# facebookresearch/sylph-few-shot-detection

Hardware: AMD Instinct MI355X
Metric: query images/sec, R50-FPN 5-way 5-shot 800x1333 (whole job) (higher is better)
Workload: dtype bf16

## Files before the change

include/sylph_hip.h:

```cpp
#ifndef SYLPH_HIP_H
#define SYLPH_HIP_H

#include <stdint.h>

#ifdef __cplusplus
extern "C" {
#endif

typedef struct sylph_ctx sylph_ctx;

enum { SYLPH_F32 = 0, SYLPH_BF16 = 1, SYLPH_F32S = 2 };

typedef struct sylph_config {
  int resnet_depth;
  int stride_in_1x1;
  int num_cls_convs;
  int num_box_convs;
  int nlevels;
  int strides[8];
  float pixel_mean[3];
  float pixel_std[3];
  int size_divisibility;
  int use_scale;
  int cond_use_bias;
// ... 60 lines not shown
int sylph_export_head(sylph_ctx* ctx, int level, float* logits_nchw_dev, float* reg_nchw_dev, float* ctr_nchw_dev,
                      float* iou_nchw_dev);

int sylph_import_head(sylph_ctx* ctx, int N, int level, const float* logits_nchw_dev, const float* reg_nchw_dev,
                      const float* ctr_nchw_dev, const float* iou_nchw_dev);

int sylph_decode_nms(sylph_ctx* ctx, const int* out_heights, const int* out_widths, int max_out, float* boxes_dev,
                     float* scores_dev, int* classes_dev, int* levels_dev, float* locations_dev, int* cand_dev,
                     int* counts_dev, int* status_dev);

int sylph_codegen(sylph_ctx* ctx, const float* boxes_dev, float* code_out_dev);
int sylph_codegen_classes(sylph_ctx* ctx, const float* boxes_dev, int shots, float* codes_out_dev);
int sylph_codegen_rois(sylph_ctx* ctx, int R, const float* boxes_dev, const int* roi_image, int n_seg, const int* seg_len,
                       float* codes_out_dev);
int sylph_roi_table_uploads(sylph_ctx* ctx, int64_t* n_out);
int sylph_codegen_weight_norm(sylph_ctx* ctx, float* weight_norm_out_dev);

int sylph_roi_align(sylph_ctx* ctx, const float* boxes_dev, float* out_nchw_dev);
int sylph_roi_align_rois(sylph_ctx* ctx, int R, const float* boxes_dev, const int* roi_image, float* out_nchw_dev);

int sylph_normalize_codes(sylph_ctx* ctx, float* codes_dev, int n, const float* weight_norm_dev);

int sylph_reduce_codes(sylph_ctx* ctx, const float* rows_dev, int n, int row_ld, float* out_dev, int num_classes,
                       int divide_by_acc);

int sylph_allgather_codes(sylph_ctx* ctx, void* comm, const float* local_dev, int n_local, int capacity, float* out_dev);
int sylph_comm_unique_id(char* id_out_128);
int sylph_comm_init_rank(sylph_ctx* ctx, const char* id_128, int nranks, int rank, void** comm_out);
int sylph_comm_destroy(void* comm);

int sylph_conv2d(sylph_ctx* ctx, const float* x_nchw_dev, int B, int C, int H, int W, const float* w_host, int Cout,
                 int KH, int KW, int stride, int pad, const float* scale_host, const float* shift_host, int relu,
                 const float* residual_nchw_dev, float* y_nchw_dev);
int sylph_group_norm(sylph_ctx* ctx, const float* x_nchw_dev, int B, int H, int W, const float* gamma_host,
                     const float* beta_host, int relu, float* y_nchw_dev);

int sylph_stem_maxpool(sylph_ctx* ctx, const float* x_nchw_dev, int B, int H, int W, const float* w_host,
                       const float* scale_host, const float* shift_host, float* stem_out_nchw_dev, float* pool_out_nchw_dev);

int sylph_set_debug_taps(sylph_ctx* ctx, int on);
int sylph_export_stage(sylph_ctx* ctx, int stage, float* out_nchw_dev);
int sylph_export_tower(sylph_ctx* ctx, int tower, int layer, int level, float* y_nchw_dev, float* coef_dev);

#define SYLPH_SUP_ROI 0
#define SYLPH_SUP_GN_Y 1
#define SYLPH_SUP_GN_COEF 2
#define SYLPH_SUP_LAYER_OUT 3
#define SYLPH_SUP_CONV_OUT 4
#define SYLPH_SUP_CONTEXT 5
#define SYLPH_SUP_MSCAM 6
#define SYLPH_SUP_TOKENS 7
#define SYLPH_SUP_CLS_TOKENS 8
int sylph_support_tap_numel(sylph_ctx* ctx, int stage, int index, int64_t* numel);
int sylph_export_support(sylph_ctx* ctx, int stage, int index, float* out_dev);

int sylph_bottleneck(sylph_ctx* ctx, const float* x_nchw_dev, int B, int Cin, int H, int W, int stride, int mid, int cout,
                     const float* const* w_host, const float* const* scale_host, const float* const* shift_host,
                     float* y_nchw_dev);
int sylph_bottleneck_even(sylph_ctx* ctx, const float* x_nchw_dev, int B, int Cin, int H, int W, int mid, int cout,
                          const float* const* w_host, const float* const* scale_host, const float* const* shift_host,
                          float* y_nchw_dev);

int sylph_fpn_lateral(sylph_ctx* ctx, const float* x_nchw_dev, int B, int C, int H, int W, const float* w_host, const float* bias_host,
                      const float* top_nchw_dev, float* y_nchw_dev);

int sylph_group_conv(sylph_ctx* ctx, const float* x_nchw_dev, int B, int C, int H, int W, int groups, int stride, const float* w_host,
// ... 24 lines not shown
```

sylph-few-shot-detection_amd/csrc/api_conv.hip:

```cpp
#include "api_internal.h"

namespace sylph_host {

void level_dims(const sylph_config& cfg, int H, int W, int* hl, int* wl, int* off, int* Ltot) {
  int h = H / 8, w = W / 8;
  int o = 0;
  for (int l = 0; l < cfg.nlevels; ++l) {
    hl[l] = h; wl[l] = w; off[l] = o;
    o += h * w;
    if (l < 2) { h = (h - 1) / 2 + 1; w = (w - 1) / 2 + 1; }
    else { h = (h + 1) / 2; w = (w + 1) / 2; }
  }
  *Ltot = o;
}

int make_geom(sylph_ctx* c, const std::vector<SegDesc>& segs, int BM, Geom* g) {
  std::vector<int2> tiles;
  for (size_t s = 0; s < segs.size(); ++s) {
    const int rows = segs[s].out_H * segs[s].out_W;
    const int t0 = (int)tiles.size();
    for (int r = 0; r < rows; r += BM) tiles.push_back(make_int2((int)s, r));
    g->seg_tiles.push_back(make_int2(t0, (int)tiles.size() - t0));
  }
  void *ds = nullptr, *dtl = nullptr;
  RET(upload(c, &ds, segs.data(), segs.size() * sizeof(SegDesc)));
  RET(upload(c, &dtl, tiles.data(), tiles.size() * sizeof(int2)));
  g->segs = (const SegDesc*)ds;
  g->tiles = (const int2*)dtl;
  g->n_mtiles = (int)tiles.size();
  return 0;
}

void pick_patch(int H, int W, int max_pos, int halo_rows, int xpad, int* ph_out, int* pw_out) {
  long best_n = -1;
  int bh = 8, bw = 16, best_halo = 0;
  for (int w = 4; w <= 32; ++w) {
    for (int h = 1; h * w <= max_pos; ++h) {
      if ((h + 2) * (w + xpad) > halo_rows) continue;
      if (((max_pos - 1) / w + 2) * (w + xpad) + (max_pos - 1) % w + 2 >= halo_rows) continue;
      const long n = (long)((H + h - 1) / h) * ((W + w - 1) / w);
      const int halo = (h + 2) * (w + 2);
      const bool better = best_n < 0 || n < best_n || (n == best_n && (halo < best_halo || (halo == best_halo && w == 16)));
      if (better) { best_n = n; bh = h; bw = w; best_halo = halo; }
    }
  }
  *ph_out = bh; *pw_out = bw;
}

void set_patch(SegDesc* s, int ph, int pw, int xpad) {
  s->ph = ph; s->pw = pw; s->hpitch = pw + xpad;
  s->inv_pw = (65536u + pw - 1) / pw;
  s->inv_hw2 = (65536u + s->hpitch - 1) / s->hpitch;
}

int make_geom_patch(sylph_ctx* c, std::vector<SegDesc> segs, int max_pos, int halo_rows, int xpad, bool pair, Geom* g, int group) {
  std::vector<int2> tiles;
  if (group < 1 || segs.size() % (size_t)group != 0) group = 1;
  size_t g0 = 0;
  bool per_image = pair && segs.size() < (1u << 20);
  for (size_t s = 0; s < segs.size(); ++s) {
    int ph, pw;
    pick_patch(segs[s].out_H, segs[s].out_W, max_pos, halo_rows, xpad, &ph, &pw);
    set_patch(&segs[s], ph, pw, xpad);
    const int t0 = (int)tiles.size();
    for (int y = 0; y < segs[s].out_H; y += ph)
      for (int x = 0; x < segs[s].out_W; x += pw) tiles.push_back(make_int2((int)s, (y << 16) | x));
    g->seg_tiles.push_back(make_int2(t0, (int)tiles.size() - t0));
    if (per_image && (s + 1) % (size_t)group == 0) {
      const size_t n = tiles.size() - g0;
      if ((n & 1) && n < 8) per_image = false;
      if (per_image) {
        if (n & 1) tiles.push_back(make_int2(0, 0x7fff << 16));
        for (size_t t = g0; t < tiles.size(); t += 2) tiles[t].x |= (int)((((t - g0) >> 1) & 0x7ff) << 20);
      }
      g0 = tiles.size();
    }
  }
  if (pair && (tiles.size() & 1)) tiles.push_back(make_int2(0, 0x7fff << 16));
  if (pair && !per_image)
    for (size_t t = 0; t < tiles.size(); t += 2) tiles[t].x |= (int)(((t >> 1) & 0x7ff) << 20);
  g->n_mtiles = (int)tiles.size();
  void *ds = nullptr, *dtl = nullptr;
  RET(upload(c, &ds, segs.data(), segs.size() * sizeof(SegDesc)));
  RET(upload(c, &dtl, tiles.data(), tiles.size() * sizeof(int2)));
  g->segs = (const SegDesc*)ds;
  g->tiles = (const int2*)dtl;
  return 0;
}

long patch_count(const std::vector<SegDesc>& segs, int max_pos, int halo_rows, int xpad) {
  long n = 0;
  for (auto& sg : segs) {
    int ph, pw;
    pick_patch(sg.out_H, sg.out_W, max_pos, halo_rows, xpad, &ph, &pw);
    n += (long)((sg.out_H + ph - 1) / ph) * ((sg.out_W + pw - 1) / pw);
  }
  return n;
}

int timed_op(sylph_ctx* c, const char* kern, double flops, hipStream_t s, const std::function<int(hipStream_t)>& fn) {
  if (!c->prof) return fn(s);
  sylph_ctx::ProfRec r;
  if (!c->prof_free.empty()) {
    r.a = c->prof_free.back().first; r.b = c->prof_free.back().second;
    c->prof_free.pop_back();
  } else {
    if (hipEventCreate(&r.a) != hipSuccess || hipEventCreate(&r.b) != hipSuccess) return -100;
  }
  r.flops = flops;
  r.kern = kern;
  (void)hipEventRecord(r.a, s);
  const int rc = fn(s);
  (void)hipEventRecord(r.b, s);
  c->prof_recs.push_back(r);
  return rc;
}

static long total_rows(const std::vector<SegDesc>& segs) {
// ... 172 lines not shown
      gsegs[i].out_row0 = r0;
      r0 += n;
      max_rows = std::max(max_rows, n);
    }
  }
  Geom g;
  if (kind == ConvKind::hpipe) RET(make_geom_patch(c, segs, 128, 256, 4, true, &g, o.segs_per_image));
  else if (kind == ConvKind::igemm_halo) RET(make_geom_patch(c, segs, 128, 184, 2, false, &g));
  else RET(make_geom(c, gsegs, BM, &g));
  ConvArgs a;
  memset(&a, 0, sizeof(a));
  a.halo = kind == ConvKind::igemm_halo;
  a.nbuf2 = r.nbuf;
  a.in = in; a.wt = L.w; a.out = out; a.res = o.res;
  if (!igemm) RET(packed_weights(c, L, r, &a));
  if (pw) {
    std::vector<PwDesc> pd;
    for (const SegDesc& sg : segs) {
      const int nrows = sg.out_H * sg.out_W;
      for (int r0 = 0; r0 < nrows; r0 += BM) {
        PwDesc d;
        memset(&d, 0, sizeof(d));
        d.row0 = r0; d.seg_rows = nrows; d.out_W = sg.out_W; d.out_row0 = sg.out_row0; d.in_row0 = sg.in_row0; d.in_W = sg.in_W;
        d.in2_row0 = sg.in2_row0; d.in2_W = o.in2 ? sg.in2_W : sg.out_W; d.res_row0 = sg.res_row0; d.res_W = sg.res_W;
        pd.push_back(d);
      }
    }
    if ((int)pd.size() != g.n_mtiles) return fail("internal: conv_pw descriptor count");
    void* pdd = nullptr;
    RET(upload(c, &pdd, pd.data(), pd.size() * sizeof(PwDesc)));
    a.pw_desc = (const PwDesc*)pdd;
  }
  a.scale = L.scale; a.shift = L.shift; a.zeros = c->zeros;
  a.segs = g.segs; a.tiles = g.tiles; a.n_mtiles = kind == ConvKind::hpipe ? (g.n_mtiles + 1) / 2 : g.n_mtiles; a.n_ntiles = L.Cout_pad / BN;
  a.Cin = L.Cin; a.Cout = o.cout_override >= 0 ? o.cout_override : L.Cout;
  a.KH = L.KH; a.KW = L.KW; a.stride = o.stride; a.pad = o.pad;
  a.in_ld = in_ld; a.out_ld = out_ld; a.res_ld = o.res_ld;
  a.relu_nch = o.relu_nch; a.mul_nch = o.mul_nch; a.res_mode = o.res_mode;
  a.stem = o.stem; a.tap_dy = o.stem ? L.Cin / 32 : 1;
  a.gn_coef = o.gn_coef; a.gn_relu = o.gn_relu;
  a.ss_padded = 1;
  if (o.in2) {
    a.in2 = o.in2; a.in2_ld = o.in2_ld; a.Cin2 = o.Cin2; a.stride2 = o.stride2;
    a.Cin = L.Cin - o.Cin2;
  }
  if (o.want_gn) {
    if (L.Cout != 256 && L.Cout != 512) return fail("fused GroupNorm statistics need Cout == 256 or 512");
    RET(c->dalloc((void**)&a.gn_partial, (size_t)(g.n_mtiles + 1) * (L.Cout / 8) * 3 * sizeof(float)));
  }
  if (geom_out) { *geom_out = g; geom_out->gn_partial = a.gn_partial; }
  const DType dt = c->dt;
  const bool of32 = o.out_f32;
  const double flops = o.flops >= 0.0 ? o.flops : 2.0 * (double)total_rows(segs) * (double)a.Cout * (double)(L.KH * L.KW) * (double)L.Cin;
  const char* kern = "conv_igemm_kernel";
  OpFn launch = [=](hipStream_t st) { return launch_conv(dt, of32, a, BM, BN, st); };
  if (kind == ConvKind::hpipe) {
    if (!conv_hpipe_ok(dt, of32, a)) return fail("internal: conv_hpipe selected for a layer it cannot run");
    kern = a.gn_coef ? "conv_hpipe_kernel<true>" : "conv_hpipe_kernel<false>";
    launch = [=](hipStream_t st) { return launch_conv_hpipe(a, st); };
  } else if (kind == ConvKind::pw) {
    if (!conv_pw_ok(dt, of32, a)) return fail("internal: conv_pw selected for a layer it cannot run");
    kern = "conv_pw_kernel";
    launch = [=](hipStream_t st) { return launch_conv_pw(a, BM, BN, st); };
  } else if (kind == ConvKind::spw) {
    if (!conv_spw_ok(dt, of32, a)) return fail("internal: conv_spw selected for a layer it cannot run");
    kern = "conv_spw_kernel";
    launch = [=](hipStream_t st) { return launch_conv_spw(a, st); };
// ... 134 lines not shown
```

sylph-few-shot-detection_amd/csrc/api_internal.h:

```cpp
#pragma once
#include <hip/hip_runtime.h>
#include <math.h>
#include <stdio.h>
#include <stdlib.h>
#include <string.h>

#include <functional>
#include <map>
#include <memory>
#include <string>
#include <tuple>
#include <vector>

#include "../../include/sylph_hip.h"
#include "common.h"
#include "kernels.h"

using namespace sylph;
namespace sylph_host {
int fail(const std::string& m);
}
using sylph_host::fail;
hipStream_t sylph_internal_stream(sylph_ctx* c);
int sylph_internal_fail(const std::string& m);
// ... 226 lines not shown
  bool stem_takes_raw = false;
  bool raw_input = false;
  std::vector<int> ep_n, ep_image;
  std::vector<int> ep_row0;
  std::vector<int2> ep_tiles32, ep_tilesBM;
  int ep_rows = 0, ep_rows_cap = 0;
  void* ep_code_w = nullptr;
  float* ep_bias = nullptr;
  int* ep_src_row = nullptr;
  int* ep_seg_row0 = nullptr;
  int2* ep_tiles_dev = nullptr;
  DecodeSeg* dsegs_ep = nullptr;
  float* bias_pad = nullptr;
  int bias_pad_cap = 0;
  ImageOut* img_out_dev = nullptr;
  ImageOut* img_out_host = nullptr;
  std::vector<ImageOut> img_out_last;
  hipEvent_t img_out_ev = nullptr;
  LevelDesc* lv_dev = nullptr;
  SupportPass sup;
  std::map<int, std::unique_ptr<SupportPass>> sup_rois;
  SupportPass* sup_last = nullptr;
};

struct OwnerScope {
  sylph_ctx* c; Plan* prev;
  OwnerScope(sylph_ctx* c_, Plan* P) : c(c_), prev(c_->alloc_owner) { c->alloc_owner = P; }
  ~OwnerScope() { c->alloc_owner = prev; }
};

struct Geom {
  const SegDesc* segs;
  const int2* tiles;
  int n_mtiles;
  std::vector<int2> seg_tiles;
  float* gn_partial = nullptr;
};

struct ConvOpts {
  int stride = 1, pad = 0;
  int relu_nch = 0, mul_nch = 0;
  const void* res = nullptr;
  int res_ld = 0, res_mode = 0;
  bool out_f32 = false;
  int cout_override = -1;
  int stem = 0;
  int want_gn = 0;
  const void* in2 = nullptr;
  int in2_ld = 0, Cin2 = 0, stride2 = 1;
  double flops = -1.0;
  const float2* gn_coef = nullptr;
  int gn_relu = 0;
  int segs_per_image = 1;
  int stream_slot = 0;
  int route_stride = 0;
};

enum class ConvKind { hpipe, igemm_halo, pw, spw, igemm_splitk, igemm };
struct ConvRoute {
  ConvKind kind = ConvKind::igemm;
  int BM = 0, BN = 0;
  int nbuf = 0;
  int ksplit = 1;
};

struct BkScratch { void *t1, *t2, *sc; void** trash; };
enum { BK_EVEN_OUT = 1, BK_IN_COMPACT = 2 };

namespace sylph_host {
std::shared_ptr<PilCoeffs> pil_bilinear_coeffs(int in_size, int out_size);
void free_plan(sylph_ctx* c, Plan* P);
int upload(sylph_ctx* c, void** dev, const void* host, size_t n);
void evict_plans(sylph_ctx* c, const Plan* keep);
void drop_plan(sylph_ctx* c, Plan* P);
Plan* get_plan(sylph_ctx* c, int B, int H, int W);
int run_ops(sylph_ctx* c, const std::vector<OpFn>& ops, const char* what);
const HostTensor* find_w(sylph_ctx* c, const std::string& k);
int pack_conv(sylph_ctx* c, const std::vector<const HostTensor*>& ws, ConvLayer* L);
int upload_vec(sylph_ctx* c, float** dev, const std::vector<float>& v, int pad_to);
int make_conv_bn(sylph_ctx* c, const std::string& name, ConvLayer* L);
int pack_conv_grouped(sylph_ctx* c, const HostTensor& w, const std::string& key, int C, int groups, const float* scale, const float* shift,
                      ConvLayer* L);
int make_conv_bias(sylph_ctx* c, const std::vector<std::string>& names, ConvLayer* L);
int make_c3sc(sylph_ctx* c, const HostTensor& w3, const float* s3, const float* h3, const HostTensor& ws, const float* ss, const float* hs, ConvLayer* L);
int make_gn(sylph_ctx* c, const std::string& name, GNLayer* G);
int upload_f32(sylph_ctx* c, const float** dev, const HostTensor* t, const std::string& what, size_t expect = 0);
int make_lin(sylph_ctx* c, const std::string& name, sylph_ctx::Lin* L);
int make_ln(sylph_ctx* c, const std::string& name, GNLayer* G);
bool has_prefix(sylph_ctx* c, const std::string& p);
void level_dims(const sylph_config& cfg, int H, int W, int* hl, int* wl, int* off, int* Ltot);
int make_geom(sylph_ctx* c, const std::vector<SegDesc>& segs, int BM, Geom* g);
void pick_patch(int H, int W, int max_pos, int halo_rows, int xpad, int* ph_out, int* pw_out);
void set_patch(SegDesc* s, int ph, int pw, int xpad);
int make_geom_patch(sylph_ctx* c, std::vector<SegDesc> segs, int max_pos, int halo_rows, int xpad, bool pair, Geom* g, int group = 1);
long patch_count(const std::vector<SegDesc>& segs, int max_pos, int halo_rows, int xpad);
int timed_op(sylph_ctx* c, const char* kern, double flops, hipStream_t s, const std::function<int(hipStream_t)>& fn);
ConvRoute pick_conv_route(const sylph_ctx* c, const ConvLayer& L, int in_ld, const std::vector<SegDesc>& segs, const ConvOpts& o);
std::string conv_route_name(const ConvRoute& r);
void adopt_records(sylph_ctx* c, sylph_ctx* tmp);
int add_conv(sylph_ctx* c, std::vector<OpFn>& ops, const ConvLayer& L, const void* in, int in_ld, void* out, int out_ld, const std::vector<SegDesc>& segs, const ConvOpts& o, Geom* geom_out = nullptr);
int add_conv_gn(sylph_ctx* c, std::vector<OpFn>& ops, const ConvLayer& L, const void* in, int in_ld, void* out, const std::vector<SegDesc>& segs, ConvOpts o, const GNLayer& G, int relu, const float2** coef_out = nullptr, OpFn* apply_out = nullptr);
int add_gn_from_partials(sylph_ctx* c, std::vector<OpFn>& ops, void* out, int ld, const std::vector<SegDesc>& segs, const Geom& g, const GNLayer& G, int relu,
                         const float2** coef_out, OpFn* apply_out, const float2** stats_out = nullptr);
int add_conv_deform(sylph_ctx* c, std::vector<OpFn>& ops, const ConvLayer& off, const ConvLayer& L, const void* in, void* out,
                    const std::vector<SegDesc>& segs, int segs_per_image, const GNLayer* G, int relu, const float2** coef_out = nullptr,
                    OpFn* apply_out = nullptr);
std::vector<SegDesc> image_segs(int B, int Hin, int Win, int Hout, int Wout, int resH = 0, int resW = 0);
int ensure_pyramid(sylph_ctx* c, Plan* P);
int add_bottleneck(sylph_ctx* c, std::vector<OpFn>& ops, const sylph_ctx::Block& blk, int B, const void* X, int Cin, int Hin, int Win, int stride, int mid, int cout, void* Y, const BkScratch& scr, int flags = 0);
bool bottleneck_takes_fuse_id(const sylph_ctx* c, const sylph_ctx::Block& blk, int B, int Cin, int Hin, int Win, int stride, int mid, int cout);
int add_conv3x3_c64(sylph_ctx* c, std::vector<OpFn>& ops, const ConvLayer& L, int B, int H, int W, const void* x, const void* res, void* y, int relu);
int add_basic_block(sylph_ctx* c, std::vector<OpFn>& ops, const sylph_ctx::Block& blk, int B, const void* X, int Cin, int Hin, int Win, int stride, int cout, void* Y, const BkScratch& scr);
int build_backbone(sylph_ctx* c, Plan* P);
std::vector<SegDesc> pyramid_segs(sylph_ctx* c, Plan* P);
int add_gn(sylph_ctx* c, Plan* P, std::vector<OpFn>& ops, void* x, const RowSeg* segs_dev, int nseg, int max_rows, const GNLayer& G, int relu);
int ensure_gn_ws(sylph_ctx* c, Plan* P, int nseg, int max_rows);
int build_head(sylph_ctx* c, Plan* P);
int build_support(sylph_ctx* c, Plan* P, SupportPass* Q);
int build_support_roienc(sylph_ctx* c, Plan* P, SupportPass* Q);
}
using namespace sylph_host;
```

sylph-few-shot-detection_amd/csrc/api_parity.hip:

```cpp
#include "api_internal.h"

extern "C" {

int sylph_conv2d(sylph_ctx* c, const float* x, int B, int C, int H, int W, const float* w_host, int Cout, int KH, int KW,
                 int stride, int pad, const float* scale_host, const float* shift_host, int relu, const float* residual,
                 float* y) {
  HIPCHK(hipSetDevice(c->device));
  const int bk = c->dt == DT_BF16 ? 64 : 32;
  if (C % bk != 0) return fail("sylph_conv2d: Cin must be a multiple of " + std::to_string(bk));
  const int Ho = (H + 2 * pad - KH) / stride + 1, Wo = (W + 2 * pad - KW) / stride + 1;
  sylph_ctx tmp;
  tmp.device = c->device; tmp.dt = c->dt; tmp.stream = c->stream; tmp.zeros = c->zeros;
  tmp.prof = c->prof;
  struct Guard { sylph_ctx* t; hipStream_t s; ~Guard() { (void)hipStreamSynchronize(s); for (void* p : t->allocs) (void)hipFree(p); } } guard{&tmp, c->stream};
  HostTensor hw;
  hw.shape = {Cout, C, KH, KW};
  hw.data.assign(w_host, w_host + (size_t)Cout * C * KH * KW);
  ConvLayer L;
  RET(pack_conv(&tmp, {&hw}, &L));
  if (scale_host) RET(upload_vec(&tmp, &L.scale, std::vector<float>(scale_host, scale_host + Cout), L.Cout_pad));
  if (shift_host) RET(upload_vec(&tmp, &L.shift, std::vector<float>(shift_host, shift_host + Cout), L.Cout_pad));
  void *xin, *yout, *res = nullptr;
  RET(tmp.dalloc(&xin, (size_t)B * H * W * C * tmp.esz()));
  RET(tmp.dalloc(&yout, (size_t)B * Ho * Wo * Cout * tmp.esz()));
  for (int b = 0; b < B; ++b)
    KCHK(launch_import_nchw(c->dt, x + (size_t)b * C * H * W, xin, C, H * W, b * H * W, C, c->stream), "import");
  ConvOpts o; o.stride = stride; o.pad = pad; o.relu_nch = relu ? (1 << 30) : 0;
  if (residual) {
    RET(tmp.dalloc(&res, (size_t)B * Ho * Wo * Cout * tmp.esz()));
    for (int b = 0; b < B; ++b)
      KCHK(launch_import_nchw(c->dt, residual + (size_t)b * Cout * Ho * Wo, res, Cout, Ho * Wo, b * Ho * Wo, Cout,
                              c->stream), "import");
    o.res = res; o.res_ld = Cout; o.res_mode = 1;
  }
  std::vector<OpFn> ops;
// ... 407 lines not shown
```

sylph-few-shot-detection_amd/csrc/common.h:

```cpp
#pragma once
#include <hip/hip_runtime.h>
#include <stdint.h>

#include <atomic>

namespace sylph {

typedef __bf16 bf16_t;
typedef __attribute__((ext_vector_type(8))) __bf16 bf16x8;
typedef __attribute__((ext_vector_type(16))) float f32x16;
typedef __attribute__((ext_vector_type(4))) float f32x4;

enum DType { DT_F32 = 0, DT_BF16 = 1, DT_F32S = 2 };

struct SegDesc {
  int in_row0, in_H, in_W;
  int out_row0, out_H, out_W;
  int res_row0, res_H, res_W;
  float mul;
  int in2_row0, in2_W;
  int ph, pw;
  int hpitch;
  unsigned inv_pw, inv_hw2;
};

struct ConvArgs {
  const void* in;
  const void* wt;
  void* out;
  const void* res;
  const float* scale;
  const float* shift;
  const void* in2;
  const void* zeros;
  const SegDesc* segs;
  const int2* tiles;
  int n_mtiles, n_ntiles;
  int Cin, Cout, KH, KW, stride, pad;
  int in_ld, out_ld, res_ld;
  int Cin2, in2_ld, stride2;
  int relu_nch;
  int mul_nch;
  int res_mode;
  float* gn_partial;
  int halo;
  int ss_padded_host;
  int ss_padded;
  int stem;
  int tap_dy;
  const float2* gn_coef;
  int gn_relu;
  void* trash;
  const struct PwDesc* pw_desc;
  const float* pw_table;
  int pw_rot_mask;
  int ksplit;
  long long split_stride;
  int nbuf2;
};

struct SplitSeg { int src_row0, dst_row0, res_row0, nrows; };

struct PwDesc { int row0, seg_rows, out_W, out_row0, in_row0, in_W, in2_row0, in2_W, res_row0, res_W, pad[6]; };

struct BkTile { int row0, H, W, yx, ph, pw; unsigned inv_pw, inv_hw2; };
struct BottleneckArgs {
  const void* x;
  void* y;
  const __bf16 *w1, *w2, *w3;
// ... 106 lines not shown
```

sylph-few-shot-detection_amd/csrc/conv_hpipe.hip:

```cpp
#include "gfx950.h"

namespace sylph {

namespace {
constexpr int PNT = 512;
constexpr int BSTAGE = 256 * 64;
constexpr int NSTAGE = 4;
constexpr int HPROWS = 256;
constexpr int HBUF = 2 * HPROWS * 64;
constexpr int HALO_OFF = NSTAGE * BSTAGE;
constexpr int COEF_OFF = HALO_OFF + 2 * HBUF;
constexpr int COEF_MAX_CIN = 512;
constexpr int LDS_BYTES = COEF_OFF + 2 * COEF_MAX_CIN * 8;
constexpr int SCP = 256 + 4;
static_assert(64 * SCP * 4 <= LDS_BYTES, "epilogue tile must fit");

constexpr int NPIECE = 2 * HPROWS / 128;
constexpr int nload(int t) { return ((t % 9 + 9) % 9) < NPIECE ? 3 : 2; }

}

template <bool GNIN>
__global__ __launch_bounds__(PNT, 1) void conv_hpipe_kernel(const ConvArgs a) {
  typedef bf16_t T;
  extern __shared__ __attribute__((aligned(16))) char smem[];

  const int L = blockIdx.x;
  const int xcd = L & 7, q0 = L >> 3;
  const int chunk = (a.n_mtiles + 7) >> 3;
  const int m_local = q0 / a.n_ntiles;
  const int nt = q0 - m_local * a.n_ntiles;
  const int mt = xcd * chunk + m_local;
  if (m_local >= chunk || mt >= a.n_mtiles) return;

  const int tid = threadIdx.x, lane = tid & 63;
  const int wave = __builtin_amdgcn_readfirstlane(tid >> 6);
  const int wm = wave >> 2, wn = wave & 3;
  const int l15 = lane & 15, lq = lane >> 4;

  int2 tl0 = a.tiles[2 * mt], tl1 = a.tiles[2 * mt + 1];
  const int rot_key = (int)((unsigned)tl0.x >> 20);
  tl0.x &= 0xfffff;
  const SegDesc sd0 = a.segs[tl0.x], sd1 = a.segs[tl1.x];

  const T* __restrict__ in = reinterpret_cast<const T*>(a.in);
  const T* __restrict__ wt = reinterpret_cast<const T*>(a.wt);
  const T* __restrict__ zero = reinterpret_cast<const T*>(a.zeros);
  const int Cin = a.Cin;
  const int ncc = Cin >> 5;
  const int c0 = (rot_key + nt) % ncc;

  const int r4 = tid >> 2, s4 = tid & 3;
  const char* hptr[NPIECE];
  unsigned hmask = 0, hcs = 0;
#pragma unroll
  for (int g = 0; g < NPIECE; ++g) {
    const bool p1 = g >= NPIECE / 2;
    const SegDesc& sd = p1 ? sd1 : sd0;
    const int ty = p1 ? tl1.y : tl0.y;
    const int h = g * 128 + r4 - (p1 ? HPROWS : 0);
    const int PW = sd.pw, HP = sd.hpitch, HR = (sd.ph + 2) * HP;
    const int hy = (int)(((unsigned)h * sd.inv_hw2) >> 16), hx = h - hy * HP;
    const int iy = (ty >> 16) - 1 + hy, ix = (ty & 0xffff) - 1 + hx;
    const bool ok = h < HR && hx < PW + 2 && (unsigned)iy < (unsigned)sd.in_H && (unsigned)ix < (unsigned)sd.in_W;
    const int cs = s4 ^ ((((hy * PW + hx) >> 2) & 1) << 1);
    hcs |= (unsigned)cs << (2 * g);
    hptr[g] = ok ? reinterpret_cast<const char*>(in + ((size_t)(sd.in_row0 + iy * sd.in_W + ix) * a.in_ld + cs * 8 + c0 * 32))
                 : reinterpret_cast<const char*>(zero + s4 * 8);
    hmask |= (ok ? 1u : 0u) << g;
  }
  const char* const wtile = reinterpret_cast<const char*>(wt) + (size_t)nt * ncc * 9 * BSTAGE;
  const unsigned wvo = (unsigned)tid * 16u;
  auto issue_halo = [&](int g, int buf) {
    char* d = smem + HALO_OFF + buf * HBUF + g * 8192 + wave * 1024;
    __builtin_amdgcn_global_load_lds((gbl_ptr_t)hptr[g], (lds_ptr_t)d, 16, 0, 0);
  };
  auto advance_halo = [&](int cc_next) {
    const int step = (c0 + cc_next == ncc) ? (32 - Cin) * 2 : 64;
#pragma unroll
    for (int g = 0; g < NPIECE; ++g) hptr[g] += ((hmask >> g) & 1u) ? step : 0;
  };
  bool w_loads = true;
  auto issue_w = [&](int stage, int j, int blk) {
    if (!w_loads) return;
    char* d = smem + stage * BSTAGE + j * 8192 + wave * 1024;
    const char* src = wtile + (size_t)blk * BSTAGE + j * 8192 + wvo;
    __builtin_amdgcn_global_load_lds((gbl_ptr_t)src, (lds_ptr_t)d, 16, 0, 0);
  };
  auto rot = [&](int cc) { const int c = c0 + cc; return c >= ncc ? c - ncc : c; };

  constexpr bool gn_in = GNIN;
  const short gn_floor = a.gn_relu != 0 ? (short)0 : (short)-32768;
  const unsigned lds0 = (unsigned)(size_t)(__attribute__((address_space(3))) char*)smem;
  u32x4 gx;
  f32x4 gc0, gc1, gc2, gc3;
  auto gn_addr = [&](int g, int cc_of_piece) { return lds0 + HALO_OFF + (cc_of_piece & 1) * HBUF + g * 8192 + tid * 16; };
  auto gn_read = [&](int g, int cc_of_piece) {
    const unsigned d = gn_addr(g, cc_of_piece);
    const int ch = rot(cc_of_piece) * 32 + (int)((hcs >> (2 * g)) & 3u) * 8;
    const unsigned cf = lds0 + COEF_OFF + ((g >= NPIECE / 2 ? Cin : 0) + ch) * 8;
    asm volatile("ds_read_b128 %0, %1" : "=v"(gx) : "v"(d));
    asm volatile("ds_read_b128 %0, %1" : "=v"(gc0) : "v"(cf));
    asm volatile("ds_read_b128 %0, %1 offset:16" : "=v"(gc1) : "v"(cf));
    asm volatile("ds_read_b128 %0, %1 offset:32" : "=v"(gc2) : "v"(cf));
    asm volatile("ds_read_b128 %0, %1 offset:48" : "=v"(gc3) : "v"(cf));
  };
  auto gn_finish = [&](int g, int cc_of_piece) {
    asm volatile("s_waitcnt lgkmcnt(0)" : "+v"(gx), "+v"(gc0), "+v"(gc1), "+v"(gc2), "+v"(gc3));
    const unsigned live = ((hmask >> g) & 1u) ? 0xffffffffu : 0u;
    const f32x4 cs[4] = {gc0, gc1, gc2, gc3};
    u32x4 y;
#pragma unroll
    for (int e = 0; e < 4; ++e) {
      const f32x2 xv = {__uint_as_float(gx[e] << 16), __uint_as_float(gx[e] & 0xffff0000u)};
      const f32x2 av = {cs[e][0], cs[e][1]}, bv = {cs[e][2], cs[e][3]};
      const f32x2 r = __builtin_elementwise_fma(xv, av, bv);
      const bf16x2 pk = __builtin_convertvector(r, bf16x2);
      const s16x2 fl = {gn_floor, gn_floor};
      const unsigned u = __builtin_bit_cast(unsigned, __builtin_elementwise_max(__builtin_bit_cast(s16x2, pk), fl));
      y[e] = u & live;
    }
    asm volatile("ds_write_b128 %0, %1" ::"v"(gn_addr(g, cc_of_piece)), "v"(y) : "memory");
  };
  auto gn_piece = [&](int g, int cc_of_piece) { gn_read(g, cc_of_piece); gn_finish(g, cc_of_piece); };

  const SegDesc& sdm = wm ? sd1 : sd0;
  const int PWm = sdm.pw, HW2m = sdm.hpitch;
  int a0[8];
#pragma unroll
  for (int i = 0; i < 8; ++i) {
    const int m = i * 16 + l15;
    const int my = (int)(((unsigned)m * sdm.inv_pw) >> 16);
    a0[i] = (wm * HPROWS + my * HW2m + (m - my * PWm)) * 64;
  }
  const int offB = (wn * 64 + l15) * 64 + ((lq ^ (((l15 >> 2) & 1) << 1)) << 4);

  f32x4 acc[8][4];
#pragma unroll
  for (int i = 0; i < 8; ++i)
#pragma unroll
    for (int j = 0; j < 4; ++j)
#pragma unroll
      for (int r = 0; r < 4; ++r) acc[i][j][r] = 0.f;
  bf16x8 fa[8], fb[4];

  auto ldfrag = [&](int cc, int t) {
    const int kh = t / 3, kw = t - 3 * kh;
    const char* bs = smem + ((cc + t) & 3) * BSTAGE;
    const char* hs = smem + HALO_OFF + (cc & 1) * HBUF + (kh * HW2m + kw) * 64;
    int key = l15;
    asm volatile("" : "+v"(key));
    const int so = (lq ^ ((((key + kh * PWm + kw) >> 2) & 1) << 1)) << 4;
#pragma unroll
    for (int j = 0; j < 4; ++j) fb[j] = *reinterpret_cast<const bf16x8*>(bs + offB + j * 1024);
#pragma unroll
    for (int i = 0; i < 8; ++i) fa[i] = *reinterpret_cast<const bf16x8*>(hs + a0[i] + so);
  };

  auto issue_next = [&](int cc, int t) {
    const int t3 = (t + 3) % 9, cc3 = cc + (t + 3) / 9;
    const int blk = cc3 < ncc ? rot(cc3) * 9 + t3 : 0;
    const int st3 = (cc + t + 3) & 3;
    if (t == 0 && cc + 1 < ncc) advance_halo(cc + 1);
    if (t < NPIECE) issue_halo(t, (cc + 1) & 1);
    issue_w(st3, 0, blk);
    issue_w(st3, 1, blk);
  };
  auto mma = [&](int cc, int t) {
    __builtin_amdgcn_s_setprio(1);
    const bool xf = gn_in && t >= 3 && t < 3 + NPIECE;
    if (xf) {
      gn_read(t - 3, cc + 1);
      sched_fence();
    }
    int n = 0;
#pragma unroll
    for (int i = 0; i < 8; ++i)
#pragma unroll
      for (int j = 0; j < 4; ++j) {
        acc[i][j] = __builtin_amdgcn_mfma_f32_16x16x32_bf16(fb[j], fa[i], acc[i][j], 0, 0, 0);
        if (xf && n == 7) {
          sched_fence();
          gn_finish(t - 3, cc + 1);
        }
        ++n;
      }
    if (xf) {
#pragma unroll
      for (int k = 0; k < 16; ++k) {
        __builtin_amdgcn_sched_group_barrier(0x008, 1, 0);
        __builtin_amdgcn_sched_group_barrier(0x002, 2, 0);
      }
    }
    __builtin_amdgcn_s_setprio(0);
  };

  auto frags_ready = [&]() {
    asm volatile("" ::"v"(fa[0]), "v"(fa[1]), "v"(fa[2]), "v"(fa[3]), "v"(fa[4]), "v"(fa[5]), "v"(fa[6]), "v"(fa[7]), "v"(fb[0]),
                 "v"(fb[1]), "v"(fb[2]), "v"(fb[3]));
  };

#pragma unroll
  for (int g = 0; g < NPIECE; ++g) issue_halo(g, 0);
#pragma unroll
  for (int t = 0; t < 3; ++t) {
    issue_w(t, 0, c0 * 9 + t);
    issue_w(t, 1, c0 * 9 + t);
  }
  if (gn_in) {
    for (int idx = tid; idx < Cin; idx += PNT) {
      const int pch = idx >= Cin / 2 ? 1 : 0, ch = (idx - pch * (Cin / 2)) * 2;
      const int seg = pch ? tl1.x : tl0.x;
      const float2 c0v = a.gn_coef[(size_t)seg * a.in_ld + ch], c1v = a.gn_coef[(size_t)seg * a.in_ld + ch + 1];
      *reinterpret_cast<float4*>(smem + COEF_OFF + (pch * Cin + ch) * 8) = make_float4(c0v.x, c1v.x, c0v.y, c1v.y);
    }
  }
  wait_vmcnt<4>();
  if (gn_in) {
    wait_lgkmcnt0();
    fenced_barrier();
#pragma unroll
    for (int g = 0; g < NPIECE; ++g) gn_piece(g, 0);
    wait_lgkmcnt0();
  }
  fenced_barrier();

#define HP_PHASE0(t)                       \
  ldfrag(cc, t);                           \
  sched_fence();                           \
  issue_next(cc, t);                       \
  wait_lgkmcnt0();                         \
  if (GNIN) frags_ready();                 \
  fenced_barrier();                        \
  mma(cc, t);                              \
  wait_vmcnt<nload((t) - 1) + nload(t)>(); \
  fenced_barrier();
#define HP_PHASE1(t)                       \
  ldfrag(cc, t);                           \
  sched_fence();                           \
  issue_next(cc, t);                       \
  wait_vmcnt<nload((t) - 1) + nload(t)>(); \
  wait_lgkmcnt0();                         \
  if (GNIN) frags_ready();                 \
  fenced_barrier();                        \
  mma(cc, t);                              \
  fenced_barrier();

  if (wm == 0) {
    for (int cc = 0; cc < ncc; ++cc) {
      HP_PHASE0(0) HP_PHASE0(1) HP_PHASE0(2) HP_PHASE0(3) HP_PHASE0(4) HP_PHASE0(5) HP_PHASE0(6) HP_PHASE0(7) HP_PHASE0(8)
    }
    fenced_barrier();
  } else {
    fenced_barrier();
    for (int cc = 0; cc < ncc; ++cc) {
      HP_PHASE1(0) HP_PHASE1(1) HP_PHASE1(2) HP_PHASE1(3) HP_PHASE1(4) HP_PHASE1(5) HP_PHASE1(6) HP_PHASE1(7) HP_PHASE1(8)
    }
  }
  wait_vmcnt<0>();
  __syncthreads();

  float* const sC = reinterpret_cast<float*>(smem);
  bf16_t* __restrict__ out = reinterpret_cast<bf16_t*>(a.out);
  const int c8 = tid & 31, rr = tid >> 5;
  const int n0 = nt * 256 + c8 * 8;
  float sc[8], sh[8];
#pragma unroll
  for (int h = 0; h < 2; ++h) {
    const float4 s4v = a.scale ? reinterpret_cast<const float4*>(a.scale + n0)[h] : make_float4(1.f, 1.f, 1.f, 1.f);
    const float4 b4v = a.shift ? reinterpret_cast<const float4*>(a.shift + n0)[h] : make_float4(0.f, 0.f, 0.f, 0.f);
    sc[4 * h] = s4v.x; sc[4 * h + 1] = s4v.y; sc[4 * h + 2] = s4v.z; sc[4 * h + 3] = s4v.w;
    sh[4 * h] = b4v.x; sh[4 * h + 1] = b4v.y; sh[4 * h + 2] = b4v.z; sh[4 * h + 3] = b4v.w;
  }
  const bool relu = a.relu_nch > 0;
#pragma unroll
  for (int pp = 0; pp < 2; ++pp) {
    const SegDesc& sp = pp ? sd1 : sd0;
    const int ty = pp ? tl1.y : tl0.y;
    const int oy0 = ty >> 16, ox0 = ty & 0xffff;
    const int PW = sp.pw, NPOS = sp.ph * sp.pw;
    bf16_t* __restrict__ outn = out + (size_t)sp.out_row0 * a.out_ld + n0;
    float gn_n = 0.f, gn_s1 = 0.f, gn_s2 = 0.f;
    const float gn_pv = sh[0];
#pragma unroll
    for (int hp = 0; hp < 2; ++hp) {
      if (pp + hp > 0) lds_barrier();
      if (wm == pp) {
#pragma unroll
        for (int ii = 0; ii < 4; ++ii)
#pragma unroll
          for (int j = 0; j < 4; ++j) {
            const f32x4& c = acc[4 * hp + ii][j];
            *reinterpret_cast<float4*>(sC + (ii * 16 + l15) * SCP + wn * 64 + j * 16 + 4 * lq) = make_float4(c[0], c[1], c[2], c[3]);
          }
      }
      lds_barrier();
#pragma unroll
      for (int it = 0; it < 4; ++it) {
        const int rl = rr + 16 * it;
        const int m = hp * 64 + rl;
        const int my = (int)(((unsigned)m * sp.inv_pw) >> 16);
        const int oy = oy0 + my, ox = ox0 + (m - my * PW);
        if (m < NPOS && oy < sp.out_H && ox < sp.out_W) {
          float v[8];
          const float4 lo = *reinterpret_cast<const float4*>(sC + rl * SCP + c8 * 8);
          const float4 hi = *reinterpret_cast<const float4*>(sC + rl * SCP + c8 * 8 + 4);
          v[0] = lo.x; v[1] = lo.y; v[2] = lo.z; v[3] = lo.w; v[4] = hi.x; v[5] = hi.y; v[6] = hi.z; v[7] = hi.w;
#pragma unroll
          for (int e = 0; e < 8; ++e) v[e] = v[e] * sc[e] + sh[e];
          if (relu) {
#pragma unroll
            for (int e = 0; e < 8; ++e) v[e] = v[e] > 0.f ? v[e] : 0.f;
          }
          if (a.gn_partial) {
#pragma unroll
            for (int e = 0; e < 8; ++e) { const float d = v[e] - gn_pv; gn_s1 += d; gn_s2 = fmaf(d, d, gn_s2); }
            gn_n += 8.f;
          }
          store8<bf16_t>(outn + (size_t)(oy * sp.out_W + ox) * a.out_ld, v);
        }
      }
    }
    if (a.gn_partial) {
      gn_n += __shfl_xor(gn_n, 32);
      gn_s1 += __shfl_xor(gn_s1, 32);
      gn_s2 += __shfl_xor(gn_s2, 32);
      lds_barrier();
      float* red = sC;
      if (lane < 32) {
        red[(wave * 32 + c8) * 3 + 0] = gn_n;
        red[(wave * 32 + c8) * 3 + 1] = gn_s1;
        red[(wave * 32 + c8) * 3 + 2] = gn_s2;
      }
      lds_barrier();
      if (tid < 32) {
// ... 56 lines not shown
```

sylph-few-shot-detection_amd/sylph_amd/_lib.py:

```python
import ctypes
import os
from ctypes import POINTER, Structure, c_char_p, c_float, c_int, c_int64, c_void_p

import torch

_HERE = os.path.dirname(os.path.abspath(__file__))
LIB_PATH = os.environ.get("SYLPH_LIB_PATH") or os.path.join(os.path.dirname(_HERE), "lib", "libsylph_hip.so")

SYLPH_F32 = 0
SYLPH_BF16 = 1
SYLPH_F32S = 2


class SylphConfig(Structure):
    _fields_ = [
        ("resnet_depth", c_int), ("stride_in_1x1", c_int), ("num_cls_convs", c_int), ("num_box_convs", c_int),
        ("nlevels", c_int), ("strides", c_int * 8), ("pixel_mean", c_float * 3), ("pixel_std", c_float * 3),
        ("size_divisibility", c_int), ("use_scale", c_int), ("cond_use_bias", c_int),
        ("pre_nms_thresh", c_float), ("pre_nms_topk", c_int), ("nms_thresh", c_float), ("post_nms_topk", c_int),
        ("thresh_with_ctr", c_int), ("quality_mode", c_int),
        ("cg_tower_layers", c_int), ("cg_has_bias", c_int), ("cg_bias_l2_norm", c_int), ("cg_post_norm", c_int),
        ("cg_conv_l2_norm", c_int), ("cg_use_weight_scale", c_int), ("prior_prob", c_float), ("cand_cap", c_int),
        ("cg_type", c_int), ("tok_num_conv", c_int), ("tok_num_fc", c_int), ("enc_layers", c_int),
        ("head_num_fc", c_int), ("head_fc_dim", c_int), ("cg_meta_bias", c_int), ("cg_has_weight", c_int), ("cg_has_scale", c_int),
# ... 8 lines not shown
    "sylph_ctx_destroy": (None, [c_void_p]),
    "sylph_last_error": (c_char_p, []),
    "sylph_set_stream": (c_int, [c_void_p, c_void_p]),
    "sylph_set_config": (c_int, [c_void_p, POINTER(SylphConfig)]),
    "sylph_load_weight": (c_int, [c_void_p, c_char_p, c_void_p, POINTER(c_int64), c_int]),
    "sylph_finalize_weights": (c_int, [c_void_p]),
    "sylph_preprocess": (c_int, [c_void_p, c_int, POINTER(c_void_p), POINTER(c_int), POINTER(c_int),
                                 POINTER(c_int), POINTER(c_int)]),
    "sylph_preprocess_u8": (c_int, [c_void_p, c_int, POINTER(c_void_p), POINTER(c_int), POINTER(c_int), POINTER(c_int),
                                    POINTER(c_int), c_int, POINTER(c_int), POINTER(c_int)]),
    "sylph_export_input": (c_int, [c_void_p, c_void_p]),
    "sylph_backbone_fpn": (c_int, [c_void_p]),
    "sylph_import_pyramid": (c_int, [c_void_p, c_int, c_int, c_int, POINTER(c_int), POINTER(c_int),
                                     POINTER(c_void_p)]),
    "sylph_export_pyramid": (c_int, [c_void_p, c_int, c_void_p]),
    "sylph_fcos_head": (c_int, [c_void_p, c_void_p, c_void_p, c_int]),
    "sylph_fcos_head_episodes": (c_int, [c_void_p, c_int, c_void_p, c_void_p, POINTER(c_int), POINTER(c_int)]),
    "sylph_fcos_head_pretrained": (c_int, [c_void_p, POINTER(c_int)]),
    "sylph_export_head": (c_int, [c_void_p, c_int, c_void_p, c_void_p, c_void_p, c_void_p]),
    "sylph_import_head": (c_int, [c_void_p, c_int, c_int, c_void_p, c_void_p, c_void_p, c_void_p]),
    "sylph_roi_align": (c_int, [c_void_p, c_void_p, c_void_p]),
    "sylph_roi_align_rois": (c_int, [c_void_p, c_int, c_void_p, POINTER(c_int), c_void_p]),
    "sylph_decode_nms": (c_int, [c_void_p, POINTER(c_int), POINTER(c_int), c_int, c_void_p, c_void_p, c_void_p,
                                 c_void_p, c_void_p, c_void_p, c_void_p, c_void_p]),
    "sylph_codegen": (c_int, [c_void_p, c_void_p, c_void_p]),
    "sylph_codegen_classes": (c_int, [c_void_p, c_void_p, c_int, c_void_p]),
    "sylph_codegen_rois": (c_int, [c_void_p, c_int, c_void_p, POINTER(c_int), c_int, POINTER(c_int), c_void_p]),
    "sylph_roi_table_uploads": (c_int, [c_void_p, POINTER(c_int64)]),
    "sylph_codegen_weight_norm": (c_int, [c_void_p, c_void_p]),
    "sylph_normalize_codes": (c_int, [c_void_p, c_void_p, c_int, c_void_p]),
    "sylph_reduce_codes": (c_int, [c_void_p, c_void_p, c_int, c_int, c_void_p, c_int, c_int]),
    "sylph_conv2d": (c_int, [c_void_p, c_void_p, c_int, c_int, c_int, c_int, c_void_p, c_int, c_int, c_int, c_int,
                             c_int, c_void_p, c_void_p, c_int, c_void_p, c_void_p]),
    "sylph_group_norm": (c_int, [c_void_p, c_void_p, c_int, c_int, c_int, c_void_p, c_void_p, c_int, c_void_p]),
    "sylph_stem_maxpool": (c_int, [c_void_p, c_void_p, c_int, c_int, c_int, c_void_p, c_void_p, c_void_p, c_void_p, c_void_p]),
    "sylph_set_debug_taps": (c_int, [c_void_p, c_int]),
    "sylph_export_stage": (c_int, [c_void_p, c_int, c_void_p]),
    "sylph_export_tower": (c_int, [c_void_p, c_int, c_int, c_int, c_void_p, c_void_p]),
    "sylph_support_tap_numel": (c_int, [c_void_p, c_int, c_int, POINTER(c_int64)]),
    "sylph_export_support": (c_int, [c_void_p, c_int, c_int, c_void_p]),
    "sylph_bottleneck": (c_int, [c_void_p, c_void_p, c_int, c_int, c_int, c_int, c_int, c_int, c_int, POINTER(c_void_p),
                                 POINTER(c_void_p), POINTER(c_void_p), c_void_p]),
    "sylph_bottleneck_even": (c_int, [c_void_p, c_void_p, c_int, c_int, c_int, c_int, c_int, c_int, POINTER(c_void_p),
                                      POINTER(c_void_p), POINTER(c_void_p), c_void_p]),
    "sylph_allgather_codes": (c_int, [c_void_p, c_void_p, c_void_p, c_int, c_int, c_void_p]),
    "sylph_comm_unique_id": (c_int, [ctypes.c_char_p]),
    "sylph_comm_init_rank": (c_int, [c_void_p, ctypes.c_char_p, c_int, c_int, POINTER(c_void_p)]),
    "sylph_comm_destroy": (c_int, [c_void_p]),
    "sylph_fpn_lateral": (c_int, [c_void_p, c_void_p, c_int, c_int, c_int, c_int, c_void_p, c_void_p, c_void_p, c_void_p]),
    "sylph_group_conv": (c_int, [c_void_p, c_void_p] + [c_int] * 6 + [c_void_p, c_void_p, c_void_p, c_int, c_void_p]),
    "sylph_bottleneck_grouped": (c_int, [c_void_p, c_void_p] + [c_int] * 8 + [POINTER(c_void_p), POINTER(c_void_p), POINTER(c_void_p),
                                                                            c_void_p]),
    "sylph_conv3x3_c64": (c_int, [c_void_p, c_void_p, c_int, c_int, c_int, c_void_p, c_void_p, c_void_p, c_int, c_void_p, c_void_p]),
    "sylph_basic_block": (c_int, [c_void_p, c_void_p] + [c_int] * 6 + [POINTER(c_void_p), POINTER(c_void_p), POINTER(c_void_p), c_void_p]),
    "sylph_device_bytes": (c_int64, [c_void_p]),
    "sylph_profile_enable": (c_int, [c_void_p, c_int]),
    "sylph_bench_conv": (c_int, [c_void_p] + [c_int] * 12 + [POINTER(c_float), POINTER(ctypes.c_double)]),
    "sylph_profile_read": (c_int, [c_void_p, POINTER(ctypes.c_double), POINTER(ctypes.c_double), POINTER(c_int64)]),
    "sylph_profile_read_kernels": (c_int, [c_void_p, c_int, ctypes.c_char_p, POINTER(ctypes.c_double), POINTER(ctypes.c_double),
                                           POINTER(c_int64), POINTER(c_int)]),
    "sylph_conv_routes_read": (c_int, [c_void_p, c_int, ctypes.c_char_p, POINTER(c_int)]),
}

_LIB = None


# ... 20 lines not shown
```

Baseline: 2362.

## Tile hpipe conv outputs as dense column-strip runs to cut padded tile waste

After: 2385 (median of 6 runs). No clear change (+1.0%).

```diff
diff --git a/include/sylph_hip.h b/include/sylph_hip.h
--- a/include/sylph_hip.h
+++ b/include/sylph_hip.h
@@ -116,6 +116,7 @@
 int sylph_conv2d(sylph_ctx* ctx, const float* x_nchw_dev, int B, int C, int H, int W, const float* w_host, int Cout,
                  int KH, int KW, int stride, int pad, const float* scale_host, const float* shift_host, int relu,
                  const float* residual_nchw_dev, float* y_nchw_dev);
+int sylph_hpipe_tiling(int H, int W, int* out, int cap, int* pw_out, int* runs_out);
 int sylph_group_norm(sylph_ctx* ctx, const float* x_nchw_dev, int B, int H, int W, const float* gamma_host,
                      const float* beta_host, int relu, float* y_nchw_dev);
 
diff --git a/sylph-few-shot-detection_amd/csrc/api_conv.hip b/sylph-few-shot-detection_amd/csrc/api_conv.hip
--- a/sylph-few-shot-detection_amd/csrc/api_conv.hip
+++ b/sylph-few-shot-detection_amd/csrc/api_conv.hip
@@ -53,37 +53,84 @@
   s->inv_hw2 = (65536u + s->hpitch - 1) / s->hpitch;
 }
 
+static bool hpipe_run_ok(int w) {
+  const int m = w - 1 + 127;
+  return (m / w + 1 + 2) * (w + 4) <= 256 && (m / w + 2) * (w + 4) + m % w + 2 < 256;
+}
+
+bool hpipe_tiling(int H, int W, std::vector<HpTile>* patches, int* ph_out, int* pw_out) {
+  int ph, pw;
+  pick_patch(H, W, 128, 256, 4, &ph, &pw);
+  long best_n = (long)((H + ph - 1) / ph) * ((W + pw - 1) / pw);
+  int rw = 0;
+  for (int w = 4; w <= 32; ++w) {
+    if (!hpipe_run_ok(w)) continue;
+    const long n = (long)((W + w - 1) / w) * (((long)H * w + 127) / 128);
+    if (n < best_n) { best_n = n; rw = w; }
+  }
+  patches->clear();
+  if (!rw) {
+    for (int y = 0; y < H; y += ph)
+      for (int x = 0; x < W; x += pw) patches->push_back(HpTile{0, (y << 16) | x, 0, ph * pw});
+    *ph_out = ph; *pw_out = pw;
+    return false;
+  }
+  int span = 1;
+  for (int x = 0; x < W; x += rw)
+    for (int p = 0; p < H * rw; p += 128) {
+      const int m0 = p % rw, count = std::min(128, H * rw - p);
+      patches->push_back(HpTile{0, ((p / rw) << 16) | x, m0, count});
+      span = std::max(span, (m0 + count - 1) / rw + 1);
+    }
+  *ph_out = span; *pw_out = rw;
+  return true;
+}
+
 int make_geom_patch(sylph_ctx* c, std::vector<SegDesc> segs, int max_pos, int halo_rows, int xpad, bool pair, Geom* g, int group) {
-  std::vector<int2> tiles;
+  std::vector<HpTile> tiles, one;
   if (group < 1 || segs.size() % (size_t)group != 0) group = 1;
   size_t g0 = 0;
   bool per_image = pair && segs.size() < (1u << 20);
+  const HpTile empty{0, 0x7fff << 16, 0, 0};
   for (size_t s = 0; s < segs.size(); ++s) {
     int ph, pw;
-    pick_patch(segs[s].out_H, segs[s].out_W, max_pos, halo_rows, xpad, &ph, &pw);
+    const int t0 = (int)tiles.size();
+    if (pair) {
+      hpipe_tiling(segs[s].out_H, segs[s].out_W, &one, &ph, &pw);
+      for (HpTile t : one) { t.seg = (int)s; tiles.push_back(t); }
+    } else {
+      pick_patch(segs[s].out_H, segs[s].out_W, max_pos, halo_rows, xpad, &ph, &pw);
+      for (int y = 0; y < segs[s].out_H; y += ph)
+        for (int x = 0; x < segs[s].out_W; x += pw) tiles.push_back(HpTile{(int)s, (y << 16) | x, 0, ph * pw});
+    }
     set_patch(&segs[s], ph, pw, xpad);
-    const int t0 = (int)tiles.size();
-    for (int y = 0; y < segs[s].out_H; y += ph)
-      for (int x = 0; x < segs[s].out_W; x += pw) tiles.push_back(make_int2((int)s, (y << 16) | x));
     g->seg_tiles.push_back(make_int2(t0, (int)tiles.size() - t0));
     if (per_image && (s + 1) % (size_t)group == 0) {
       const size_t n = tiles.size() - g0;
       if ((n & 1) && n < 8) per_image = false;
       if (per_image) {
-        if (n & 1) tiles.push_back(make_int2(0, 0x7fff << 16));
-        for (size_t t = g0; t < tiles.size(); t += 2) tiles[t].x |= (int)((((t - g0) >> 1) & 0x7ff) << 20);
+        if (n & 1) tiles.push_back(empty);
+        for (size_t t = g0; t < tiles.size(); t += 2) tiles[t].seg |= (int)((((t - g0) >> 1) & 0x7ff) << 20);
       }
       g0 = tiles.size();
     }
   }
-  if (pair && (tiles.size() & 1)) tiles.push_back(make_int2(0, 0x7fff << 16));
+  if (pair && (tiles.size() & 1)) tiles.push_back(empty);
   if (pair && !per_image)
-    for (size_t t = 0; t < tiles.size(); t += 2) tiles[t].x |= (int)(((t >> 1) & 0x7ff) << 20);
+    for (size_t t = 0; t < tiles.size(); t += 2) tiles[t].seg |= (int)(((t >> 1) & 0x7ff) << 20);
   g->n_mtiles = (int)tiles.size();
   void *ds = nullptr, *dtl = nullptr;
   RET(upload(c, &ds, segs.data(), segs.size() * sizeof(SegDesc)));
-  RET(upload(c, &dtl, tiles.data(), tiles.size() * sizeof(int2)));
   g->segs = (const SegDesc*)ds;
+  if (pair) {
+    RET(upload(c, &dtl, tiles.data(), tiles.size() * sizeof(HpTile)));
+    g->tiles = nullptr;
+    g->hp_tiles = (const HpTile*)dtl;
+    return 0;
+  }
+  std::vector<int2> t2;
+  for (const HpTile& t : tiles) t2.push_back(make_int2(t.seg, t.yx));
+  RET(upload(c, &dtl, t2.data(), t2.size() * sizeof(int2)));
   g->tiles = (const int2*)dtl;
   return 0;
 }
@@ -322,7 +369,7 @@
     a.pw_desc = (const PwDesc*)pdd;
   }
   a.scale = L.scale; a.shift = L.shift; a.zeros = c->zeros;
-  a.segs = g.segs; a.tiles = g.tiles; a.n_mtiles = kind == ConvKind::hpipe ? (g.n_mtiles + 1) / 2 : g.n_mtiles; a.n_ntiles = L.Cout_pad / BN;
+  a.segs = g.segs; a.tiles = g.tiles; a.hp_tiles = g.hp_tiles; a.n_mtiles = kind == ConvKind::hpipe ? (g.n_mtiles + 1) / 2 : g.n_mtiles; a.n_ntiles = L.Cout_pad / BN;
   a.Cin = L.Cin; a.Cout = o.cout_override >= 0 ? o.cout_override : L.Cout;
   a.KH = L.KH; a.KW = L.KW; a.stride = o.stride; a.pad = o.pad;
   a.in_ld = in_ld; a.out_ld = out_ld; a.res_ld = o.res_ld;
diff --git a/sylph-few-shot-detection_amd/csrc/api_internal.h b/sylph-few-shot-detection_amd/csrc/api_internal.h
--- a/sylph-few-shot-detection_amd/csrc/api_internal.h
+++ b/sylph-few-shot-detection_amd/csrc/api_internal.h
@@ -282,6 +282,7 @@
 struct Geom {
   const SegDesc* segs;
   const int2* tiles;
+  const HpTile* hp_tiles = nullptr;
   int n_mtiles;
   std::vector<int2> seg_tiles;
   float* gn_partial = nullptr;
@@ -342,6 +343,7 @@
 int make_geom(sylph_ctx* c, const std::vector<SegDesc>& segs, int BM, Geom* g);
 void pick_patch(int H, int W, int max_pos, int halo_rows, int xpad, int* ph_out, int* pw_out);
 void set_patch(SegDesc* s, int ph, int pw, int xpad);
+bool hpipe_tiling(int H, int W, std::vector<HpTile>* patches, int* ph_out, int* pw_out);
 int make_geom_patch(sylph_ctx* c, std::vector<SegDesc> segs, int max_pos, int halo_rows, int xpad, bool pair, Geom* g, int group = 1);
 long patch_count(const std::vector<SegDesc>& segs, int max_pos, int halo_rows, int xpad);
 int timed_op(sylph_ctx* c, const char* kern, double flops, hipStream_t s, const std::function<int(hipStream_t)>& fn);
diff --git a/sylph-few-shot-detection_amd/csrc/api_parity.hip b/sylph-few-shot-detection_amd/csrc/api_parity.hip
--- a/sylph-few-shot-detection_amd/csrc/api_parity.hip
+++ b/sylph-few-shot-detection_amd/csrc/api_parity.hip
@@ -1,6 +1,19 @@
 #include "api_internal.h"
 
 extern "C" {
+
+int sylph_hpipe_tiling(int H, int W, int* out, int cap, int* pw_out, int* runs_out) {
+  if (H < 1 || W < 1 || H > 0x7ffe || W > 0xffff) return -1;
+  std::vector<sylph::HpTile> t;
+  int ph = 0, pw = 0;
+  const bool runs = sylph_host::hpipe_tiling(H, W, &t, &ph, &pw);
+  for (size_t i = 0; i < t.size() && (int)i < cap; ++i) {
+    out[4 * i] = t[i].yx >> 16; out[4 * i + 1] = t[i].yx & 0xffff; out[4 * i + 2] = t[i].m0; out[4 * i + 3] = t[i].count;
+  }
+  if (pw_out) *pw_out = pw;
+  if (runs_out) *runs_out = runs ? 1 : 0;
+  return (int)t.size();
+}
 
 int sylph_conv2d(sylph_ctx* c, const float* x, int B, int C, int H, int W, const float* w_host, int Cout, int KH, int KW,
                  int stride, int pad, const float* scale_host, const float* shift_host, int relu, const float* residual,
diff --git a/sylph-few-shot-detection_amd/csrc/common.h b/sylph-few-shot-detection_amd/csrc/common.h
--- a/sylph-few-shot-detection_amd/csrc/common.h
+++ b/sylph-few-shot-detection_amd/csrc/common.h
@@ -24,6 +24,12 @@
   unsigned inv_pw, inv_hw2;
 };
 
+struct HpTile {
+  int seg;
+  int yx;
+  int m0, count;
+};
+
 struct ConvArgs {
   const void* in;
   const void* wt;
@@ -35,6 +41,7 @@
   const void* zeros;
   const SegDesc* segs;
   const int2* tiles;
+  const HpTile* hp_tiles;
   int n_mtiles, n_ntiles;
   int Cin, Cout, KH, KW, stride, pad;
   int in_ld, out_ld, res_ld;
diff --git a/sylph-few-shot-detection_amd/csrc/conv_hpipe.hip b/sylph-few-shot-detection_amd/csrc/conv_hpipe.hip
--- a/sylph-few-shot-detection_amd/csrc/conv_hpipe.hip
+++ b/sylph-few-shot-detection_amd/csrc/conv_hpipe.hip
@@ -38,10 +38,11 @@
   const int wm = wave >> 2, wn = wave & 3;
   const int l15 = lane & 15, lq = lane >> 4;
 
-  int2 tl0 = a.tiles[2 * mt], tl1 = a.tiles[2 * mt + 1];
-  const int rot_key = (int)((unsigned)tl0.x >> 20);
-  tl0.x &= 0xfffff;
-  const SegDesc sd0 = a.segs[tl0.x], sd1 = a.segs[tl1.x];
+  HpTile tl0 = a.hp_tiles[2 * mt];
+  const HpTile tl1 = a.hp_tiles[2 * mt + 1];
+  const int rot_key = (int)((unsigned)tl0.seg >> 20);
+  tl0.seg &= 0xfffff;
+  const SegDesc sd0 = a.segs[tl0.seg], sd1 = a.segs[tl1.seg];
 
   const T* __restrict__ in = reinterpret_cast<const T*>(a.in);
   const T* __restrict__ wt = reinterpret_cast<const T*>(a.wt);
@@ -57,9 +58,12 @@
   for (int g = 0; g < NPIECE; ++g) {
     const bool p1 = g >= NPIECE / 2;
     const SegDesc& sd = p1 ? sd1 : sd0;
-    const int ty = p1 ? tl1.y : tl0.y;
+    const HpTile& tl = p1 ? tl1 : tl0;
+    const int ty = tl.yx;
     const int h = g * 128 + r4 - (p1 ? HPROWS : 0);
-    const int PW = sd.pw, HP = sd.hpitch, HR = (sd.ph + 2) * HP;
+    const int PW = sd.pw, HP = sd.hpitch;
+    const int span = (int)(((unsigned)(max(tl.m0 + tl.count, 1) - 1) * sd.inv_pw) >> 16) + 1;
+    const int HR = (span + 2) * HP;
     const int hy = (int)(((unsigned)h * sd.inv_hw2) >> 16), hx = h - hy * HP;
     const int iy = (ty >> 16) - 1 + hy, ix = (ty & 0xffff) - 1 + hx;
     const bool ok = h < HR && hx < PW + 2 && (unsigned)iy < (unsigned)sd.in_H && (unsigned)ix < (unsigned)sd.in_W;
@@ -126,10 +130,11 @@
 
   const SegDesc& sdm = wm ? sd1 : sd0;
   const int PWm = sdm.pw, HW2m = sdm.hpitch;
+  const int m0m = wm ? tl1.m0 : tl0.m0;
   int a0[8];
 #pragma unroll
   for (int i = 0; i < 8; ++i) {
-    const int m = i * 16 + l15;
+    const int m = m0m + i * 16 + l15;
     const int my = (int)(((unsigned)m * sdm.inv_pw) >> 16);
     a0[i] = (wm * HPROWS + my * HW2m + (m - my * PWm)) * 64;
   }
@@ -150,7 +155,7 @@
     const char* hs = smem + HALO_OFF + (cc & 1) * HBUF + (kh * HW2m + kw) * 64;
     int key = l15;
     asm volatile("" : "+v"(key));
-    const int so = (lq ^ ((((key + kh * PWm + kw) >> 2) & 1) << 1)) << 4;
+    const int so = (lq ^ ((((key + (m0m + kh * PWm + kw)) >> 2) & 1) << 1)) << 4;
 #pragma unroll
     for (int j = 0; j < 4; ++j) fb[j] = *reinterpret_cast<const bf16x8*>(bs + offB + j * 1024);
 #pragma unroll
@@ -210,7 +215,7 @@
   if (gn_in) {
     for (int idx = tid; idx < Cin; idx += PNT) {
       const int pch = idx >= Cin / 2 ? 1 : 0, ch = (idx - pch * (Cin / 2)) * 2;
-      const int seg = pch ? tl1.x : tl0.x;
+      const int seg = pch ? tl1.seg : tl0.seg;
       const float2 c0v = a.gn_coef[(size_t)seg * a.in_ld + ch], c1v = a.gn_coef[(size_t)seg * a.in_ld + ch + 1];
       *reinterpret_cast<float4*>(smem + COEF_OFF + (pch * Cin + ch) * 8) = make_float4(c0v.x, c1v.x, c0v.y, c1v.y);
     }
@@ -276,9 +281,9 @@
 #pragma unroll
   for (int pp = 0; pp < 2; ++pp) {
     const SegDesc& sp = pp ? sd1 : sd0;
-    const int ty = pp ? tl1.y : tl0.y;
-    const int oy0 = ty >> 16, ox0 = ty & 0xffff;
-    const int PW = sp.pw, NPOS = sp.ph * sp.pw;
+    const HpTile& tp = pp ? tl1 : tl0;
+    const int oy0 = tp.yx >> 16, ox0 = tp.yx & 0xffff;
+    const int PW = sp.pw, M0 = tp.m0, NPOS = tp.count;
     bf16_t* __restrict__ outn = out + (size_t)sp.out_row0 * a.out_ld + n0;
     float gn_n = 0.f, gn_s1 = 0.f, gn_s2 = 0.f;
     const float gn_pv = sh[0];
@@ -298,9 +303,9 @@
 #pragma unroll
       for (int it = 0; it < 4; ++it) {
         const int rl = rr + 16 * it;
-        const int m = hp * 64 + rl;
-        const int my = (int)(((unsigned)m * sp.inv_pw) >> 16);
-        const int oy = oy0 + my, ox = ox0 + (m - my * PW);
+        const int m = hp * 64 + rl, ms = M0 + m;
+        const int my = (int)(((unsigned)ms * sp.inv_pw) >> 16);
+        const int oy = oy0 + my, ox = ox0 + (ms - my * PW);
         if (m < NPOS && oy < sp.out_H && ox < sp.out_W) {
           float v[8];
           const float4 lo = *reinterpret_cast<const float4*>(sC + rl * SCP + c8 * 8);
diff --git a/sylph-few-shot-detection_amd/sylph_amd/_lib.py b/sylph-few-shot-detection_amd/sylph_amd/_lib.py
--- a/sylph-few-shot-detection_amd/sylph_amd/_lib.py
+++ b/sylph-few-shot-detection_amd/sylph_amd/_lib.py
@@ -64,6 +64,7 @@
     "sylph_reduce_codes": (c_int, [c_void_p, c_void_p, c_int, c_int, c_void_p, c_int, c_int]),
     "sylph_conv2d": (c_int, [c_void_p, c_void_p, c_int, c_int, c_int, c_int, c_void_p, c_int, c_int, c_int, c_int,
                              c_int, c_void_p, c_void_p, c_int, c_void_p, c_void_p]),
+    "sylph_hpipe_tiling": (c_int, [c_int, c_int, POINTER(c_int), c_int, POINTER(c_int), POINTER(c_int)]),
     "sylph_group_norm": (c_int, [c_void_p, c_void_p, c_int, c_int, c_int, c_void_p, c_void_p, c_int, c_void_p]),
     "sylph_stem_maxpool": (c_int, [c_void_p, c_void_p, c_int, c_int, c_int, c_void_p, c_void_p, c_void_p, c_void_p, c_void_p]),
     "sylph_set_debug_taps": (c_int, [c_void_p, c_int]),
```
